# m4rch1n0/vqvae

Hardware: AMD Instinct MI355X
Metric: latents/sec through geodesic kNN+APSP+K-medoids (higher is better)
Workload: dtype f64-exact(u32 fixed point)

## Files before the change

vqvae_amd/csrc/common.hip:

```cpp
#include "geo_common.h"

#include <cstdlib>
#include <cstring>

namespace geo {

namespace {
struct OptionName { const char *name, *env; int Options::*field; };
const OptionName kOptionNames[] = {
    {"sssp_sb", "GEO_SSSP_SB", &Options::sssp_sb},
    {"sssp_act", "GEO_SSSP_ACT", &Options::sssp_act},
    {"sssp_sparse_div", "GEO_SSSP_SPARSE_DIV", &Options::sssp_sparse_div},
    {"sssp_map_div", "GEO_SSSP_MAP_DIV", &Options::sssp_map_div},
    {"sssp_group", "GEO_SSSP_GROUP", &Options::sssp_group},
    {"sssp_grouped_cap", "GEO_SSSP_GROUPED_CAP", &Options::sssp_grouped_cap},
    {"sssp_trace", "GEO_SSSP_TRACE", &Options::sssp_trace},
    {"sssp_u32", "GEO_SSSP_U32", &Options::sssp_u32},
    {"sssp_push", "GEO_SSSP_PUSH", &Options::sssp_push},
    {"sssp_order", "GEO_SSSP_ORDER", &Options::sssp_order},
    {"sssp_delta", "GEO_SSSP_DELTA", &Options::sssp_delta},
    {"sssp_push_blocks", "GEO_SSSP_PUSH_BLOCKS", &Options::sssp_push_blocks},
    {"knn_filter", "GEO_KNN_FILTER", &Options::knn_filter},
    {"kpp_grid", "GEO_KPP_GRID", &Options::kpp_grid},
    {"kpp_profile", "GEO_KPP_PROFILE", &Options::kpp_profile},
    {"jvp_mid", "GEO_JVP_MID", &Options::jvp_mid},
    {"jvp_back_valu", "GEO_JVP_BACK_VALU", &Options::jvp_back_valu},
    {"jvp_front_valu", "GEO_JVP_FRONT_VALU", &Options::jvp_front_valu},
    {"jvp_per_node", "GEO_JVP_PER_NODE", &Options::jvp_per_node},
    {"jvp_node_jacobian", "GEO_JVP_NODE_JACOBIAN", &Options::jvp_node_jacobian},
    {"jvp_pipe_grid", "GEO_JVP_PIPE_GRID", &Options::jvp_pipe_grid},
};
Options from_environment() {
    Options o;
    for (const OptionName &e : kOptionNames) {
        const char *v = getenv(e.env);
        if (!v) continue;
        if (e.field == &Options::jvp_mid) o.jvp_mid = v[0] == 'f' ? 1 : (v[0] == 'c' ? 2 : (v[0] == 'a' ? 3 : atoi(v)));
        else o.*(e.field) = atoi(v);
    }
    return o;
}
}

Options &options() {
    static Options o = from_environment();
    return o;
}

static thread_local char g_err[512] = "";

void set_error(const char *fmt, ...) {
    va_list ap;
    va_start(ap, fmt);
    vsnprintf(g_err, sizeof(g_err), fmt, ap);
    va_end(ap);
}

constexpr int SCAN_THREADS = 256;
constexpr int SCAN_ITEMS = 8;
constexpr int SCAN_TILE = SCAN_THREADS * SCAN_ITEMS;

__global__ __launch_bounds__(SCAN_THREADS) void scan_tiles_kernel(const int32_t *__restrict__ in,
                                                                 int32_t *__restrict__ out,
// ... 114 lines not shown
```

vqvae_amd/csrc/geo_common.h:

```cpp
#pragma once
#include <hip/hip_runtime.h>

#include <cstdarg>
#include <cstdint>
#include <cstdio>

#include "geo_hip.h"

namespace geo {

void set_error(const char *fmt, ...);

#define GEO_HIP_CHECK(expr)                                                                      \
    do {                                                                                         \
        hipError_t _e = (expr);                                                                  \
        if (_e != hipSuccess) {                                                                  \
            geo::set_error("%s failed: %s (%s:%d)", #expr, hipGetErrorString(_e), __FILE__, __LINE__); \
            return GEO_E_HIP;                                                                    \
        }                                                                                        \
    } while (0)

#define GEO_REQUIRE(cond, ...)              \
    do {                                    \
        if (!(cond)) {                      \
            geo::set_error(__VA_ARGS__);    \
            return GEO_E_ARG;               \
        }                                   \
    } while (0)

#define GEO_LAUNCH_CHECK() GEO_HIP_CHECK(hipGetLastError())

struct Options {
    int sssp_sb = -1, sssp_act = 1, sssp_sparse_div = -1, sssp_map_div = -1, sssp_group = 1, sssp_grouped_cap = 256,
        sssp_trace = 0, sssp_u32 = 1, sssp_push = 1 ,
        sssp_delta = 8 , sssp_order = 0 , sssp_push_blocks = 64, knn_filter = 1, kpp_grid = 256, kpp_profile = 0, jvp_mid = 0 ,
        jvp_back_valu = 0, jvp_front_valu = 0, jvp_per_node = 1 ,
        jvp_pipe_grid = 1 ,
        jvp_node_jacobian = 1 ;
};
Options &options();

static inline size_t align_up(size_t x, size_t a = 256) { return (x + a - 1) / a * a; }

struct Arena {
    char *base;
    size_t size, off;
    Arena(void *p, size_t n) : base(static_cast<char *>(p)), size(n), off(0) {}
    template <typename T>
    T *take(size_t count) {
        size_t bytes = align_up(count * sizeof(T));
        if (off + bytes > size) return nullptr;
        T *r = reinterpret_cast<T *>(base + off);
        off += bytes;
        return r;
    }
};

size_t scan_tmp_bytes(int64_t n);
int exclusive_scan_i32(const int32_t *in, int32_t *out, int64_t n, void *tmp, size_t tmp_bytes,
                       int64_t *total_host, hipStream_t stream);

static inline int grid_for(int64_t work_items, int per_block, int cap = 8192) {
    int64_t g = (work_items + per_block - 1) / per_block;
    if (g < 1) g = 1;
    if (g > cap) g = cap;
    return static_cast<int>(g);
}

}
```

vqvae_amd/csrc/jvp.hip:

```cpp
#include "geo_common.h"

#include <cmath>
#include <cstdlib>
#include <type_traits>
#include <vector>

namespace {

constexpr int TS = 32;
constexpr int NC = 128;
constexpr int MAX_BLOCKS = 4;
constexpr int FRONT_MAX_N1 = 1024;
constexpr int BACK_TS = 8;

typedef float f32x16 __attribute__((ext_vector_type(16)));
typedef __bf16 bf16x8 __attribute__((ext_vector_type(8)));
typedef unsigned short u16x8 __attribute__((ext_vector_type(8)));

struct Shape {
    int d, c0, c1, c2, co, s_out, pad3, p_out;
    int n1, n2;
    int opix_per_chunk, n_chunks;
};

// ... 855 lines not shown
#pragma unroll
    for (int lc = 0; lc < NL; ++lc) {
        const int ch = wg == 0 ? MidGeom::chunk_of(0, lc) : MidGeom::chunk_of(1, lc);
        const int op = lo == 0 ? MidGeom::opix(ch, 0) : MidGeom::opix(ch, 1);
#pragma unroll
        for (int q = 0; q < 16; ++q) {
            const int row = (q & 3) + 8 * (q >> 2) + 4 * (lane >> 5);
            const float x = accp[lc][q] + bias, t = acct[lc][q];
            if (!TONLY) pre2[(slot0 + row) * n2 + (size_t)op * c2 + co] = x;
            tpre2[(slot0 + row) * n2 + (size_t)op * c2 + co] = t;
            if (!TONLY && row < n_valid) { sx += x; sxx += (double)x * x; st_ += t; sxt += (double)x * t; }
        }
    }
    if (want_stats) {
        sx += __shfl_xor(sx, 32, 64); sxx += __shfl_xor(sxx, 32, 64);
        st_ += __shfl_xor(st_, 32, 64); sxt += __shfl_xor(sxt, 32, 64);
        if (lane < 32) { red[wave][lane][0] = sx; red[wave][lane][1] = sxx; red[wave][lane][2] = st_; red[wave][lane][3] = sxt; }
        __syncthreads();
        if (threadIdx.x < 64) {
            const int w0 = threadIdx.x >> 5, l = threadIdx.x & 31;
            double a0 = 0, a1 = 0, a2 = 0, a3 = 0;
#pragma unroll
            for (int w = 0; w < 4; ++w) { a0 += red[w0 + 2 * w][l][0]; a1 += red[w0 + 2 * w][l][1]; a2 += red[w0 + 2 * w][l][2]; a3 += red[w0 + 2 * w][l][3]; }
            double *p = partial2 + ((size_t)tile * c2 + threadIdx.x) * 4;
            p[0] = a0; p[1] = a1; p[2] = a2; p[3] = a3;
        }
    }
#ifdef GEO_MID_PROF
    { const unsigned long long t_e = __builtin_amdgcn_s_memtime();
      GEO_MP_ADD(6, t_e - mp_prev); GEO_MP_ADD(5, mp_wait); GEO_MP_ADD(7, 1); }
#endif
}

__global__ __launch_bounds__(512, 2) void mid_pipe_kernel(const float *__restrict__ pre1, const float *__restrict__ tpre1,
                                                         const NormConst *__restrict__ consts1, int consts_per_group,
                                                         int tiles_per_group, int n_tiles, int ,
                                                         const unsigned short *__restrict__ B3, const float *__restrict__ b2,
                                                         float *__restrict__ pre2, float *__restrict__ tpre2,
                                                         double *__restrict__ partial2, int want_stats, int64_t e_base,
                                                         int64_t n_edges, int batch) {
    constexpr int C1 = 128, LDK = C1 + 8, KS = C1 / 16, NL = 4, c2 = 64;
    typedef float f32x2 __attribute__((ext_vector_type(2)));
    __shared__ __attribute__((aligned(16))) unsigned short A3[2][3][2][TS][LDK];
    const int lane = threadIdx.x & 63, wave = __builtin_amdgcn_readfirstlane((int)(threadIdx.x >> 6));
    const int wq = wave & 3, wg = wave >> 2;
    constexpr int n1 = 4 * C1, n2 = 16 * c2;
    const int r = lane & 31, h = lane >> 5;
    const int k0p = 2 * lane;
    const int lo = wq >> 1, co = (wq & 1) * 32 + r;
    const float bias = b2[co];
    const unsigned v_out = (unsigned)(4 * h * n2 + co) * 4u;
    const int my_tiles = (n_tiles - (int)blockIdx.x + (int)gridDim.x - 1) / (int)gridDim.x;
    if (my_tiles <= 0) return;

    f32x16 accp[NL], acct[NL];
    auto zero_acc = [&]() {
#pragma unroll
        for (int lc = 0; lc < NL; ++lc)
#pragma unroll
            for (int i = 0; i < 16; ++i) { accp[lc][i] = 0.f; acct[lc][i] = 0.f; }
    };
    zero_acc();
    NormConst kA, kB;
    f32x2 rp[4], rt[4];
    auto load_consts = [&](int tile) {
        const NormConst *kp = consts1 + (size_t)(consts_per_group ? tile / tiles_per_group : 0) * C1 + k0p;
        kA = kp[0];
        kB = kp[1];
    };
    const unsigned v_pair = (unsigned)k0p * 4u;
    auto fetch = [&](int tile, int px, int sample0, auto ns_tag) {
        constexpr int NS = decltype(ns_tag)::value;
        const size_t tbase = (size_t)tile * TS * n1;
        const __amdgpu_buffer_rsrc_t rp_src = __builtin_amdgcn_make_buffer_rsrc(const_cast<float *>(pre1 + tbase), 0, TS * n1 * 4, 0x00020000);
        const __amdgpu_buffer_rsrc_t rt_src = __builtin_amdgcn_make_buffer_rsrc(const_cast<float *>(tpre1 + tbase), 0, TS * n1 * 4, 0x00020000);
        const int soff = (sample0 * n1 + MidGeom::pix(px) * C1) * 4;
#pragma unroll
        for (int i = 0; i < NS; ++i) {
            rp[i] = __builtin_bit_cast(f32x2, __builtin_amdgcn_raw_buffer_load_b64(rp_src, v_pair, soff + i * n1 * 4, 0));
            rt[i] = __builtin_bit_cast(f32x2, __builtin_amdgcn_raw_buffer_load_b64(rt_src, v_pair, soff + i * n1 * 4, 0));
        }
        __builtin_amdgcn_sched_group_barrier(0x020, 2 * NS, 0);
    };
    auto stage = [&](int buf, int sample0, auto ns_tag) {
        constexpr int NS = decltype(ns_tag)::value;
        unsigned w_idx = (unsigned)((buf * 3 * 2 * TS + sample0) * LDK + k0p);
        asm volatile("" : "+v"(w_idx));
        unsigned short *w = &A3[0][0][0][0][0] + w_idx;
#pragma unroll
        for (int i = 0; i < NS; ++i) {
            float a0, t0, a1, t1;
            norm_relu(kA, rp[i].x, rt[i].x, &a0, &t0);
            norm_relu(kB, rp[i].y, rt[i].y, &a1, &t1);
            unsigned wa[3], wt[3];
            split3_pair(a0, a1, wa[0], wa[1], wa[2]);
            split3_pair(t0, t1, wt[0], wt[1], wt[2]);
#pragma unroll
            for (int part = 0; part < 3; ++part) {
                *reinterpret_cast<unsigned *>(w + (part * 2 + 0) * TS * LDK + i * LDK) = wa[part];
                *reinterpret_cast<unsigned *>(w + (part * 2 + 1) * TS * LDK + i * LDK) = wt[part];
            }
        }
    };
    std::integral_constant<int, 4> HALF;
    const int s_half = 4 * wave, s_full = 8 * wq;

    bf16x8 ring[3][3];
    const unsigned b_lane = (unsigned)(h * 3 * NC * 8 + (wq * 32 + r) * 8) * 2u;
    const __amdgpu_buffer_rsrc_t b_rsrc = __builtin_amdgcn_make_buffer_rsrc(
        const_cast<unsigned short *>(B3), 0, (int)((size_t)8 * MAX_BLOCKS * C1 * NC * 3 * 2), 0x00020000);
    auto ring_init = [&]() {
        const int cb0 = wg == 0 ? MidGeom::prod_cb(0, MidGeom::pix(0), 0) : MidGeom::prod_cb(1, MidGeom::pix(0), 0);
        const int cb1 = wg == 0 ? MidGeom::prod_cb(0, MidGeom::pix(0), 1) : MidGeom::prod_cb(1, MidGeom::pix(0), 1);
#pragma unroll
        for (int part = 0; part < 3; ++part) {
            ring[0][part] = __builtin_bit_cast(bf16x8, __builtin_amdgcn_raw_buffer_load_b128(b_rsrc, b_lane, (cb0 * KS * 2 * 3 + part) * NC * 8 * 2, 0));
            ring[1][part] = __builtin_bit_cast(bf16x8, __builtin_amdgcn_raw_buffer_load_b128(b_rsrc, b_lane, (cb1 * KS * 2 * 3 + part) * NC * 8 * 2, 0));
        }
    };
    auto epilogue = [&](int tile) {
        const int group = tile / tiles_per_group;
        int64_t cnt_g = n_edges - (e_base + (int64_t)(group >> 1) * batch);
        if (cnt_g > batch) cnt_g = batch;
        const int n_valid = (int)cnt_g - (tile - group * tiles_per_group) * TS;
        const size_t tbase = (size_t)tile * TS * n2;
        const __amdgpu_buffer_rsrc_t p_dst = __builtin_amdgcn_make_buffer_rsrc(pre2 + tbase, 0, TS * n2 * 4, 0x00020000);
        const __amdgpu_buffer_rsrc_t t_dst = __builtin_amdgcn_make_buffer_rsrc(tpre2 + tbase, 0, TS * n2 * 4, 0x00020000);
        double sx = 0, sxx = 0, st_ = 0, sxt = 0;
#pragma unroll
        for (int lc = 0; lc < NL; ++lc) {
            const int ch = wg == 0 ? MidGeom::chunk_of(0, lc) : MidGeom::chunk_of(1, lc);
            const int op = lo == 0 ? MidGeom::opix(ch, 0) : MidGeom::opix(ch, 1);
#pragma unroll
            for (int q = 0; q < 16; ++q) {
                const int row = (q & 3) + 8 * (q >> 2) + 4 * h;
                const float x = accp[lc][q] + bias, t = acct[lc][q];
                const int soff = (((q & 3) + 8 * (q >> 2)) * n2 + op * c2) * 4;
                __builtin_amdgcn_raw_buffer_store_b32(__float_as_uint(x), p_dst, v_out, soff, 0);
                __builtin_amdgcn_raw_buffer_store_b32(__float_as_uint(t), t_dst, v_out, soff, 0);
                const double xd = row < n_valid ? (double)x : 0.0, td = row < n_valid ? (double)t : 0.0;
                sx += xd; sxx = fma(xd, xd, sxx); st_ += td; sxt = fma(xd, td, sxt);
            }
        }
        if (want_stats) {
            sx += __shfl_xor(sx, 32, 64); sxx += __shfl_xor(sxx, 32, 64);
            st_ += __shfl_xor(st_, 32, 64); sxt += __shfl_xor(sxt, 32, 64);
            if (lane < 32) {
                double *pp = partial2 + (((size_t)tile * 4 + (wg * 2 + (wq >> 1))) * c2 + co) * 4;
                pp[0] = sx; pp[1] = sxx; pp[2] = st_; pp[3] = sxt;
            }
        }
        zero_acc();
    };

    const unsigned short *a3 = &A3[0][0][0][0][0];
    const unsigned a_lane = (unsigned)(r * LDK + h * 8);
    constexpr unsigned A_BUF = 3u * 2u * TS * LDK;
#define GEO_PIPE_PIXEL(WGV, IPV)                                                                                       \
    mid_products<C1, false, WGV, IPV>(a3, a_lane + ((IPV) & 1) * A_BUF, b_rsrc, b_lane, accp, acct, ring)

#define GEO_PIPE_SEP() __builtin_amdgcn_sched_barrier(0)
#define GEO_STAGE_FULL(BUF, TILE, PX)                                                                                   \
    { stage(BUF, s_full, HALF); fetch(TILE, PX, s_full + 4, HALF); GEO_PIPE_SEP(); stage(BUF, s_full + 4, HALF); }

    int tile = blockIdx.x;
    load_consts(tile);
    fetch(tile, 0, s_half, HALF);
    ring_init();
    stage(0, s_half, HALF);
    if (wg == 0) fetch(tile, 1, s_full, HALF);
    else fetch(tile, 2, s_half, HALF);
    if (wg == 0) __builtin_amdgcn_s_setprio(1);
    lds_barrier();
#ifdef GEO_MID_PROF
    unsigned long long pb_prev = __builtin_amdgcn_s_memtime(), pb_wait = 0;
#define GEO_PB(slot)                                                                                                   \
    { const unsigned long long t_a = __builtin_amdgcn_s_memtime();                                                      \
      lds_barrier();                                                                                                    \
      const unsigned long long t_b = __builtin_amdgcn_s_memtime();                                                      \
      if (lane == 0 && wq == 0) { atomicAdd(&g_mid_prof[wg][1 + slot], t_a - pb_prev); atomicAdd(&g_mid_prof[wg][5], t_b - t_a);   \
                                  if (slot == 3) atomicAdd(&g_mid_prof[wg][7], 1ull); }                                 \
      pb_prev = t_b; }
#else
#define GEO_PB(slot) lds_barrier();
// ... 8 lines not shown
            GEO_PIPE_PIXEL(0, 2); GEO_PIPE_SEP(); stage(1, s_half, HALF); GEO_PB(2);
            GEO_PIPE_PIXEL(0, 3); GEO_PIPE_SEP();
            epilogue(tile);
            GEO_PIPE_SEP();
            if (has_next) { load_consts(next); fetch(next, 1, s_full, HALF); ring_init(); }
            GEO_PB(3);
            tile = next;
        }
    } else {
        for (int it = 0; it < my_tiles; ++it) {
            const int next = tile + (int)gridDim.x;
            const bool has_next = it + 1 < my_tiles;
            if (it > 0) { epilogue(tile - (int)gridDim.x); GEO_PIPE_SEP(); ring_init(); }
            GEO_PIPE_PIXEL(1, 0); GEO_PB(0);
            stage(0, s_half, HALF); fetch(tile, 3, s_half, HALF); GEO_PIPE_SEP();
            GEO_PIPE_PIXEL(1, 1); GEO_PB(1);
            stage(1, s_half, HALF);
            if (has_next) { load_consts(next); fetch(next, 0, s_full, HALF); }
            GEO_PIPE_SEP();
            GEO_PIPE_PIXEL(1, 2); GEO_PB(2);
            if (has_next) { GEO_STAGE_FULL(0, next, 0); fetch(next, 2, s_half, HALF); }
            GEO_PIPE_SEP();
            GEO_PIPE_PIXEL(1, 3); GEO_PB(3);
            tile = next;
        }
        epilogue(tile - (int)gridDim.x);
    }
#undef GEO_STAGE_FULL
#undef GEO_PIPE_SEP
#undef GEO_PB
#undef GEO_PIPE_PIXEL
}

__global__ __launch_bounds__(256) void slot_valid_kernel(int64_t e_base, int64_t n_edges, int batch, int tiles_per_group,
                                                        int64_t n_slots, int32_t *__restrict__ slot_valid) {
    for (int64_t i = (int64_t)blockIdx.x * blockDim.x + threadIdx.x; i < n_slots; i += (int64_t)gridDim.x * blockDim.x) {
        const int64_t per_group = (int64_t)tiles_per_group * TS;
        const int64_t g = i / per_group, within = i % per_group;
        const int64_t e = e_base + (g >> 1) * batch + within;
        slot_valid[i] = (within < batch && e < n_edges) ? 1 : 0;
    }
}

__global__ __launch_bounds__(256) void slot_node_kernel(const int32_t *__restrict__ src, const int32_t *__restrict__ dst,
                                                       int64_t e_base, int64_t n_edges, int batch, int tiles_per_group,
                                                       int64_t n_slots, int32_t *__restrict__ slot_node) {
    for (int64_t i = (int64_t)blockIdx.x * blockDim.x + threadIdx.x; i < n_slots; i += (int64_t)gridDim.x * blockDim.x) {
        const int64_t per_group = (int64_t)tiles_per_group * TS;
        const int64_t g = i / per_group, within = i % per_group;
        const int64_t e = e_base + (g >> 1) * batch + within;
        slot_node[i] = (within < batch && e < n_edges) ? ((g & 1) ? dst[e] : src[e]) : 0;
    }
}

__global__ __launch_bounds__(256) void back_kernel(const float *__restrict__ pre2, const float *__restrict__ tpre2,
                                                  const NormConst *__restrict__ consts2, int consts_per_group,
                                                  int slots_per_group, int c2, int co_n, int s_out, int pad3,
                                                  const float *__restrict__ W3p, const float *__restrict__ b3,
                                                  float *__restrict__ norms) {
    extern __shared__ __attribute__((aligned(16))) float smem[];
    const int n2 = 16 * c2;
    const int p_out = co_n * s_out * s_out;
    const int ldc = c2 + 4;
    const int lds_n2 = 16 * ldc;
    float *a2 = smem;
    float *ta2 = a2 + (size_t)BACK_TS * lds_n2;
// ... 63 lines not shown
}

__global__ __launch_bounds__(256) void pack_back_bf16_kernel(const float *__restrict__ w3, int c2, int co_n, int s_out,
                                                            int pad3, int np, unsigned short *__restrict__ W3b) {
    const int K = 16 * c2, P = co_n * s_out * s_out;
    const size_t total = (size_t)K * np;
    for (size_t i = (size_t)blockIdx.x * blockDim.x + threadIdx.x; i < total; i += (size_t)gridDim.x * blockDim.x) {
        const int o = (int)(i % np), k = (int)(i / np);
        float v = 0.f;
        if (o < P) {
            const int ip = k / c2, ci = k % c2, iy = ip >> 2, ix = ip & 3;
            const int co = o / (s_out * s_out), oy = (o / s_out) % s_out, ox = o % s_out;
            const int ky = oy + pad3 - 2 * iy, kx = ox + pad3 - 2 * ix;
            if (ky >= 0 && ky < 4 && kx >= 0 && kx < 4) v = w3[(((size_t)ci * co_n + co) * 4 + ky) * 4 + kx];
        }
        unsigned short q[3];
        split3(v, q[0], q[1], q[2]);
        const int kb = k >> 7, kk = k & 127, ks = kk >> 4, h = (kk >> 3) & 1, j = kk & 7;
        for (int part = 0; part < 3; ++part)
            W3b[((((size_t)kb * 3 + part) * 8 + ks) * 2 + h) * (size_t)np * 8 + (size_t)o * 8 + j] = q[part];
    }
}

template <int NT, bool GN, int MODE = 0>
__global__ __launch_bounds__(256, 2) void back_mfma_kernel(const float *__restrict__ pre2, const float *__restrict__ tpre2,
                                                       const NormConst *__restrict__ consts2, int consts_per_group,
                                                       int tiles_per_group, int co_n, int s_out,
                                                       const unsigned short *__restrict__ W3b,
                                                       const float *__restrict__ b3, float *__restrict__ norms,
                                                       const float4 *__restrict__ gs2, float *__restrict__ sg_node = nullptr,
                                                       const int32_t *__restrict__ src = nullptr,
                                                       const int32_t *__restrict__ dst = nullptr, int64_t e_base = 0,
                                                       int64_t n_edges = 0, int batch = 1, float *__restrict__ jac_node = nullptr,
                                                       int unit_d = 0) {
    constexpr int C2 = 64, KB = 128, LDK = KB + 8, NP = NT * 32;
    __shared__ __attribute__((aligned(16))) unsigned short A3[3][2][TS][LDK];
    __shared__ NormConst kc[C2];
    __shared__ float4 gsl[GN ? TS : 1][32];
    const int tile = blockIdx.x;
    const int group = tile / tiles_per_group;
    const int lane = threadIdx.x & 63, wave = threadIdx.x >> 6;
    const int n2 = 16 * C2, P = co_n * s_out * s_out;
    const size_t slot0 = (size_t)tile * TS;
    for (int c = threadIdx.x; c < C2; c += 256) kc[c] = consts2[(size_t)(consts_per_group ? group : 0) * C2 + c];
    if (GN)
        for (int i = threadIdx.x; i < TS * 32; i += 256) gsl[i >> 5][i & 31] = gs2[slot0 * 32 + i];

    f32x16 accp[NT], acct[NT];
#pragma unroll
    for (int nt = 0; nt < NT; ++nt)
#pragma unroll
        for (int i = 0; i < 16; ++i) { accp[nt][i] = 0.f; acct[nt][i] = 0.f; }

    const int r = lane & 31, h = lane >> 5;
    const int ss = threadIdx.x >> 3, k0 = (threadIdx.x & 7) * 16;
    auto edge_of = [&](int sample) -> int64_t {
        const int tg = tile - group * tiles_per_group;
        const int64_t e = e_base + (int64_t)(group >> 1) * batch + (int64_t)tg * TS + sample;
        return (tg * TS + sample >= batch || e >= n_edges) ? -1 : e;
    };
    auto node_of = [&](int sample) -> size_t {
        const int64_t e = edge_of(sample);
        return e < 0 ? 0 : (size_t)((group & 1) ? dst[e] : src[e]);
    };
    const size_t prow = MODE == 1 ? node_of(ss) : slot0 + ss;
    for (int kb = 0; kb < 8; ++kb) {
        __syncthreads();
        {
            const float *xp = pre2 + prow * n2 + (size_t)kb * KB + k0;
            const float *xt = (MODE == 2 ? pre2 : tpre2) + (slot0 + ss) * n2 + (size_t)kb * KB + k0;
#pragma unroll
            for (int k8 = 0; k8 < 16; k8 += 8) {
                u16x8 pp[3], pt[3];
#pragma unroll
                for (int k = 0; k < 8; ++k) {
                    float a, ta;
                    const int c = (k0 + k8 + k) & (C2 - 1);
                    if (GN) norm_relu_gn(gsl[GN ? ss : 0][c >> 1], kc[c].sc, kc[c].beta, xp[k8 + k], xt[k8 + k], &a, &ta);
                    else norm_relu(kc[c], xp[k8 + k], xt[k8 + k], &a, &ta);
                    unsigned short q1, q2, q3;
                    if (MODE != 1) { split3(a, q1, q2, q3); pp[0][k] = q1; pp[1][k] = q2; pp[2][k] = q3; }
                    if (MODE != 2) { split3(ta, q1, q2, q3); pt[0][k] = q1; pt[1][k] = q2; pt[2][k] = q3; }
                }
#pragma unroll
                for (int part = 0; part < 3; ++part) {
                    if (MODE != 1) *reinterpret_cast<u16x8 *>(&A3[part][0][ss][k0 + k8]) = pp[part];
                    if (MODE != 2) *reinterpret_cast<u16x8 *>(&A3[part][1][ss][k0 + k8]) = pt[part];
                }
            }
        }
        __syncthreads();
#pragma unroll
        for (int kq = 0; kq < 2; ++kq) {
            const int ks = wave * 2 + kq;
            bf16x8 ap[3], at[3];
#pragma unroll
            for (int part = 0; part < 3; ++part) {
                if (MODE != 1) ap[part] = *reinterpret_cast<const bf16x8 *>(&A3[part][0][r][ks * 16 + h * 8]);
                if (MODE != 2) at[part] = *reinterpret_cast<const bf16x8 *>(&A3[part][1][r][ks * 16 + h * 8]);
            }
#pragma unroll
            for (int nt = 0; nt < NT; ++nt) {
                bf16x8 b[3];
#pragma unroll
                for (int part = 0; part < 3; ++part)
                    b[part] = *reinterpret_cast<const bf16x8 *>(
                        W3b + ((((size_t)kb * 3 + part) * 8 + ks) * 2 + h) * (size_t)NP * 8 + (size_t)(nt * 32 + r) * 8);
                if (MODE != 1) accp[nt] = __builtin_amdgcn_mfma_f32_32x32x16_bf16(ap[2], b[0], accp[nt], 0, 0, 0);
                if (MODE != 2) acct[nt] = __builtin_amdgcn_mfma_f32_32x32x16_bf16(at[2], b[0], acct[nt], 0, 0, 0);
                if (MODE != 1) accp[nt] = __builtin_amdgcn_mfma_f32_32x32x16_bf16(ap[0], b[2], accp[nt], 0, 0, 0);
                if (MODE != 2) acct[nt] = __builtin_amdgcn_mfma_f32_32x32x16_bf16(at[0], b[2], acct[nt], 0, 0, 0);
                if (MODE != 1) accp[nt] = __builtin_amdgcn_mfma_f32_32x32x16_bf16(ap[1], b[1], accp[nt], 0, 0, 0);
                if (MODE != 2) acct[nt] = __builtin_amdgcn_mfma_f32_32x32x16_bf16(at[1], b[1], acct[nt], 0, 0, 0);
                if (MODE != 1) accp[nt] = __builtin_amdgcn_mfma_f32_32x32x16_bf16(ap[1], b[0], accp[nt], 0, 0, 0);
                if (MODE != 2) acct[nt] = __builtin_amdgcn_mfma_f32_32x32x16_bf16(at[1], b[0], acct[nt], 0, 0, 0);
                if (MODE != 1) accp[nt] = __builtin_amdgcn_mfma_f32_32x32x16_bf16(ap[0], b[1], accp[nt], 0, 0, 0);
                if (MODE != 2) acct[nt] = __builtin_amdgcn_mfma_f32_32x32x16_bf16(at[0], b[1], acct[nt], 0, 0, 0);
                if (MODE != 1) accp[nt] = __builtin_amdgcn_mfma_f32_32x32x16_bf16(ap[0], b[0], accp[nt], 0, 0, 0);
                if (MODE != 2) acct[nt] = __builtin_amdgcn_mfma_f32_32x32x16_bf16(at[0], b[0], acct[nt], 0, 0, 0);
            }
        }
    }
    float *red = reinterpret_cast<float *>(&A3[0][0][0][0]);
    const int row = threadIdx.x >> 3, c4 = (threadIdx.x & 7) * 4;
    const size_t nrow = MODE == 1 ? node_of(row) : slot0 + row;
    float *jrow = nullptr;
    if (MODE == 1 && jac_node) {
        const int64_t e = edge_of(row);
        if (e >= 0) jrow = jac_node + (nrow * unit_d + (size_t)(e % unit_d)) * NP;
    }
    double sumsq = 0.0;
#pragma unroll
    for (int nt = 0; nt < NT; ++nt) {
        __syncthreads();
#pragma unroll
        for (int q = 0; q < 16; ++q) {
            const int rr = (q & 3) + 8 * (q >> 2) + 4 * (lane >> 5);
            if (MODE != 1) red[((wave * 2 + 0) * 32 + rr) * 33 + (lane & 31)] = accp[nt][q];
            if (MODE != 2) red[((wave * 2 + 1) * 32 + rr) * 33 + (lane & 31)] = acct[nt][q];
        }
        __syncthreads();
#pragma unroll
        for (int c = 0; c < 4; ++c) {
            const int o = nt * 32 + c4 + c;
            if (o < P) {
                float x = b3[o / (s_out * s_out)], t = 0.f;
#pragma unroll
                for (int w = 0; w < 4; ++w) {
                    if (MODE != 1) x += red[((w * 2 + 0) * 32 + row) * 33 + c4 + c];
                    if (MODE != 2) t += red[((w * 2 + 1) * 32 + row) * 33 + c4 + c];
                }
                const float sg = MODE == 1 ? sg_node[nrow * NP + o] : 1.0f / (1.0f + expf(-x));
                if (MODE == 2) sg_node[nrow * NP + o] = sg;
                const float j = t * sg * (1.0f - sg);
                if (MODE == 1 && jrow) jrow[o] = j;
                sumsq += (double)(j * j);
            }
        }
    }
    sumsq += __shfl_xor(sumsq, 1, 64);
    sumsq += __shfl_xor(sumsq, 2, 64);
    sumsq += __shfl_xor(sumsq, 4, 64);
    if (MODE != 2 && (threadIdx.x & 7) == 0) norms[slot0 + row] = (float)sqrt(sumsq);
}

__global__ __launch_bounds__(256) void combine_kernel(const float *__restrict__ norms, int64_t e_base, int64_t e_count,
                                                     int batch, int slots_per_group, float *__restrict__ len_out) {
    for (int64_t i = (int64_t)blockIdx.x * blockDim.x + threadIdx.x; i < e_count; i += (int64_t)gridDim.x * blockDim.x) {
        const int64_t chunk = i / batch, within = i % batch;
        const float a = norms[(chunk * 2 + 0) * slots_per_group + within];
        const float b = norms[(chunk * 2 + 1) * slots_per_group + within];
        len_out[e_base + i] = 0.5f * (a + b);
    }
}

__global__ __launch_bounds__(256) void pair_edges_kernel(int64_t n_nodes, int d, int64_t n_pseudo, int32_t *__restrict__ src,
                                                        int32_t *__restrict__ dst) {
    for (int64_t i = (int64_t)blockIdx.x * blockDim.x + threadIdx.x; i < n_pseudo; i += (int64_t)gridDim.x * blockDim.x) {
        const int64_t a = 2 * (i / d), b = a + 1 < n_nodes ? a + 1 : n_nodes - 1;
        src[i] = (int32_t)a;
        dst[i] = (int32_t)b;
    }
}

__global__ __launch_bounds__(256) void jacobian_lengths_kernel(const float *__restrict__ z, const int32_t *__restrict__ src,
                                                              const int32_t *__restrict__ dst, int64_t n_edges, int d, int p_out,
                                                              int np, const float *__restrict__ jac_node,
                                                              float *__restrict__ len_out) {
    const int64_t gid = (int64_t)blockIdx.x * 256 + threadIdx.x;
    const int l = (int)(gid & 15);
    int64_t e = gid >> 4;
    const bool live = e < n_edges;
    if (!live) e = n_edges - 1;
    const int64_t a = src[e], b = dst[e];
    float dz[16];
#pragma unroll
// ... 272 lines not shown
        const bool front_mfma = s.d > 16 && s.n1 % 32 == 0 && geo::options().jvp_front_valu == 0;
        if (s.d <= 16) { if (geo::options().jvp_front_valu == 2 && s.n1 % 32 == 0 && !unit_d) GEO_FRONT_MFMA(16); else GEO_FRONT(16); }
        else if (s.d <= 32) { if (front_mfma) GEO_FRONT_MFMA(32); else GEO_FRONT(32); }
        else { if (front_mfma) GEO_FRONT_MFMA(64); else GEO_FRONT(64); }
#undef GEO_FRONT_MFMA
#undef GEO_FRONT
        GEO_LAUNCH_CHECK();
        if (batch_stats) {
            finalize_batch_kernel<<<geo::grid_for(p_groups * s.c1, 256), 256, 0, stream>>>(
                part1, pl.tiles_per_group, 1, 4, s.c1, e_base, n_edges, batch, dc->g1, dc->be1, dc->eps, k1, (int)p_groups,
                track ? stats : nullptr);
            if (track)
                running_update_kernel<<<(unsigned)((s.c1 + 7) / 8), 256, 0, stream>>>(stats, (int)p_groups, s.c1, dc->momentum,
                                                                          const_cast<float *>(dc->rm1), const_cast<float *>(dc->rv1));
            GEO_LAUNCH_CHECK();
        }
        if (gs1) {
            group_stats_kernel<<<geo::grid_for(p_slots * 32, 256), 256, 0, stream>>>(pre1, tpre1, p_slots, 4, s.c1, 32,
                                                                                    dc->eps, gs1);
            GEO_LAUNCH_CHECK();
        }
        const dim3 mgrid((unsigned)p_tiles, (unsigned)s.n_chunks);
#define GEO_MID(C1V)                                                                                               \
    mid_kernel<C1V><<<mgrid, 256, 0, stream>>>(pre1, tpre1, k1, batch_stats ? 1 : 0, pl.tiles_per_group, tab,       \
                                               s.opix_per_chunk, s.c2, B2p, dc->b2, pre2, tpre2, part2,             \
                                               batch_stats ? 1 : 0, slot_valid)
#define GEO_MID3(C1V)                                                                                              \
    mid_bf16_kernel<C1V><<<mgrid, 256, 0, stream>>>(pre1, tpre1, k1, batch_stats ? 1 : 0, pl.tiles_per_group, tab,  \
                                                    s.opix_per_chunk, s.c2, B3, dc->b2, pre2, tpre2, part2,        \
                                                    batch_stats ? 1 : 0, slot_valid)
        const bool mid_all = mid_split && s.n_chunks == 8 && s.opix_per_chunk == 2 && s.c1 >= 32 &&
                             mid_opt != 2;
        const bool mid_pipe = mid_all && !per_node && !gs1 && s.c1 == 128 && s.c2 == 64 && mid_opt != 3;
        if (mid_all && per_node) {
#define GEO_MIDA_T(C1V, GNV)                                                                                       \
    mid_all_kernel<C1V, GNV, true><<<(unsigned)p_tiles, 512, 0, stream>>>(pre1, tpre1, k1, 0, pl.tiles_per_group,       \
                                                                          s.c2, B3, dc->b2, pre2, tpre2, part2, 0,     \
                                                                          slot_valid, gs1, e_base, n_edges, batch)
            if (gs1) { if (s.c1 == 128) GEO_MIDA_T(128, true); else if (s.c1 == 64) GEO_MIDA_T(64, true); else GEO_MIDA_T(32, true); }
            else if (s.c1 == 128) GEO_MIDA_T(128, false);
            else if (s.c1 == 64) GEO_MIDA_T(64, false);
            else GEO_MIDA_T(32, false);
#undef GEO_MIDA_T
        } else if (mid_pipe) {
            static int n_cu = 0;
            if (n_cu == 0) {
                int devid = 0;
                hipDeviceProp_t prop;
                GEO_HIP_CHECK(hipGetDevice(&devid));
                GEO_HIP_CHECK(hipGetDeviceProperties(&prop, devid));
                n_cu = prop.multiProcessorCount > 0 ? prop.multiProcessorCount : 256;
            }
            const int per_cu = geo::options().jvp_pipe_grid > 0 ? geo::options().jvp_pipe_grid : 1;
            const unsigned pgrid = (unsigned)std::min<int64_t>(p_tiles, (int64_t)n_cu * per_cu);
            mid_pipe_kernel<<<pgrid, 512, 0, stream>>>(pre1, tpre1, k1, batch_stats ? 1 : 0, pl.tiles_per_group, (int)p_tiles,
                                                       s.c2, B3, dc->b2, pre2, tpre2, part2, batch_stats ? 1 : 0, e_base,
                                                       n_edges, batch);
        } else if (mid_all) {
#define GEO_MIDA(C1V, GNV)                                                                                         \
    mid_all_kernel<C1V, GNV><<<(unsigned)p_tiles, 512, 0, stream>>>(pre1, tpre1, k1, batch_stats ? 1 : 0,           \
                                                                    pl.tiles_per_group, s.c2, B3, dc->b2,           \
                                                                    pre2, tpre2, part2, batch_stats ? 1 : 0,        \
                                                                    slot_valid, gs1, e_base, n_edges, batch)
            if (gs1) {
                if (s.c1 == 128) GEO_MIDA(128, true);
                else if (s.c1 == 64) GEO_MIDA(64, true);
                else GEO_MIDA(32, true);
            } else if (s.c1 == 128) GEO_MIDA(128, false);
            else if (s.c1 == 64) GEO_MIDA(64, false);
            else GEO_MIDA(32, false);
#undef GEO_MIDA
        } else if (mid_split) {
            if (s.c1 == 128) GEO_MID3(128);
            else if (s.c1 == 64) GEO_MID3(64);
            else GEO_MID3(32);
        } else {
            if (s.c1 == 128) GEO_MID(128);
            else if (s.c1 == 64) GEO_MID(64);
            else GEO_MID(32);
        }
#undef GEO_MID3
#undef GEO_MID
        GEO_LAUNCH_CHECK();
        if (batch_stats) {
            finalize_batch_kernel<<<geo::grid_for(p_groups * s.c2, 256), 256, 0, stream>>>(
                part2, pl.tiles_per_group, mid_pipe ? 4 : (mid_all ? 1 : 16), 16, s.c2, e_base, n_edges, batch, dc->g2, dc->be2, dc->eps, k2, (int)p_groups,
                track ? stats : nullptr);
            if (track)
                running_update_kernel<<<(unsigned)((s.c2 + 7) / 8), 256, 0, stream>>>(stats, (int)p_groups, s.c2, dc->momentum,
                                                                          const_cast<float *>(dc->rm2), const_cast<float *>(dc->rv2));
            GEO_LAUNCH_CHECK();
        }
        if (gs2 && per_node) {
            slot_node_kernel<<<geo::grid_for(p_slots, 256), 256, 0, stream>>>(src, dst, e_base, n_edges, batch, pl.tiles_per_group,
                                                                             p_slots, slot_valid);
            group_stats_kernel<<<geo::grid_for(p_slots * 32, 256), 256, 0, stream>>>(pre2_node, tpre2, p_slots, 16, s.c2, 32,
                                                                                    dc->eps, gs2, slot_valid);
            GEO_LAUNCH_CHECK();
        } else if (gs2) {
            group_stats_kernel<<<geo::grid_for(p_slots * 32, 256), 256, 0, stream>>>(pre2, tpre2, p_slots, 16, s.c2, 32,
                                                                                    dc->eps, gs2);
            GEO_LAUNCH_CHECK();
        }
#define GEO_BACK(NTV, GNV)                                                                                         \
    back_mfma_kernel<NTV, GNV><<<(unsigned)p_tiles, 256, 0, stream>>>(pre2, tpre2, k2, batch_stats ? 1 : 0,         \
                                                                      pl.tiles_per_group, s.co, s.s_out, W3b,       \
                                                                      dc->b3, norms, gs2)
#define GEO_BACK_T(NTV, GNV)                                                                                       \
    back_mfma_kernel<NTV, GNV, 1><<<(unsigned)p_tiles, 256, 0, stream>>>(pre2_node, tpre2, k2, 0, pl.tiles_per_group, s.co, \
                                                                         s.s_out, W3b, dc->b3, norms, gs2, sg_node, src,   \
                                                                         dst, e_base, n_edges, batch, jac_node, unit_d)
        if (per_node && back_nt == 1) { if (gs2) GEO_BACK_T(1, true); else GEO_BACK_T(1, false); }
        else if (per_node) { if (gs2) GEO_BACK_T(6, true); else GEO_BACK_T(6, false); }
#undef GEO_BACK_T
        else if (back_mfma && back_nt == 1) { if (gs2) GEO_BACK(1, true); else GEO_BACK(1, false); }
        else if (back_mfma) { if (gs2) GEO_BACK(6, true); else GEO_BACK(6, false); }
#undef GEO_BACK
        else
            back_kernel<<<(unsigned)(p_slots / BACK_TS), 256, back_lds, stream>>>(
                pre2, tpre2, k2, batch_stats ? 1 : 0, pl.slots_per_group, s.c2, s.co, s.s_out, s.pad3, W3p, dc->b3, norms);
        GEO_LAUNCH_CHECK();
        if (len_out) {
            combine_kernel<<<geo::grid_for(e_count, 256), 256, 0, stream>>>(norms, e_base, e_count, batch,
                                                                            pl.slots_per_group, len_out);
            GEO_LAUNCH_CHECK();
        }
    }
    return GEO_OK;
}

struct JacobianPlan {
    int64_t n_pseudo;
    size_t np, extra_bytes, bytes;
};

bool node_jacobian_plan(const geo_decoder_desc *dc, int64_t n_nodes, int64_t n_edges, int batch, JacobianPlan *jp) {
    const geo::Options &o = geo::options();
    Shape s;
    if (!dc || n_nodes <= 0 || n_edges <= 0 || !make_shape(dc, &s)) return false;
    if (o.jvp_node_jacobian == 0 || o.jvp_per_node == 0 || o.jvp_back_valu || o.jvp_mid == 1 || o.jvp_mid == 2) return false;
    if (dc->norm == 1 && dc->bn_train) return false;
    if (s.d > 16 || s.c1 % 16 != 0 || s.c1 < 32 || s.c2 != 64 || s.n_chunks != 8 || s.opix_per_chunk != 2) return false;
    const int back_nt = (s.p_out + 31) / 32;
    if (back_nt != 1 && back_nt != 6) return false;
    if (o.jvp_node_jacobian == 1 && 4 * n_edges < 3 * n_nodes * s.d) return false;
// ... 78 lines not shown
```

Measured before the change: 2.102 million.

## Deduplicate repeated start-node rows in JVP mid and back stages

Adds a run-detection kernel that finds consecutive edges sharing the same source node, then computes the primal mid/back activations once per unique start node instead of once per edge. The generic pipe kernel handles only end-node tiles, and a new mid_start kernel processes the compacted start rows plus a per-tile tangent pass that gathers primal values through a row map. The back stage is split into three launches (end side, compact start primal, start tangent via row_map). This removes redundant work when edges are sorted by source, at the cost of extra launches, scratch space reused from part1/pre1, and a single-block-per-chunk serial loop for compact rows.

```diff
diff --git a/vqvae_amd/csrc/common.hip b/vqvae_amd/csrc/common.hip
--- a/vqvae_amd/csrc/common.hip
+++ b/vqvae_amd/csrc/common.hip
@@ -29,6 +29,7 @@
     {"jvp_per_node", "GEO_JVP_PER_NODE", &Options::jvp_per_node},
     {"jvp_node_jacobian", "GEO_JVP_NODE_JACOBIAN", &Options::jvp_node_jacobian},
     {"jvp_pipe_grid", "GEO_JVP_PIPE_GRID", &Options::jvp_pipe_grid},
+    {"jvp_start_dedup", "GEO_JVP_START_DEDUP", &Options::jvp_start_dedup},
 };
 Options from_environment() {
     Options o;
diff --git a/vqvae_amd/csrc/geo_common.h b/vqvae_amd/csrc/geo_common.h
--- a/vqvae_amd/csrc/geo_common.h
+++ b/vqvae_amd/csrc/geo_common.h
@@ -36,7 +36,8 @@
         sssp_delta = 8 , sssp_order = 0 , sssp_push_blocks = 64, knn_filter = 1, kpp_grid = 256, kpp_profile = 0, jvp_mid = 0 ,
         jvp_back_valu = 0, jvp_front_valu = 0, jvp_per_node = 1 ,
         jvp_pipe_grid = 1 ,
-        jvp_node_jacobian = 1 ;
+        jvp_node_jacobian = 1 ,
+        jvp_start_dedup = 1 ;
 };
 Options &options();
 
diff --git a/vqvae_amd/csrc/jvp.hip b/vqvae_amd/csrc/jvp.hip
--- a/vqvae_amd/csrc/jvp.hip
+++ b/vqvae_amd/csrc/jvp.hip
@@ -911,6 +911,21 @@
 #endif
 }
 
+struct Bn2Sums { double sx = 0, sxx = 0, st = 0, sxt = 0; };
+__device__ __forceinline__ void bn2_add(Bn2Sums &a, float x, float t, bool live) {
+    const double xd = live ? (double)x : 0.0, td = live ? (double)t : 0.0;
+    a.sx += xd; a.sxx = fma(xd, xd, a.sxx); a.st += td; a.sxt = fma(xd, td, a.sxt);
+}
+__device__ __forceinline__ void bn2_store(Bn2Sums a, double *__restrict__ partial2, int tile, int wslot, int co, int lane) {
+    a.sx += __shfl_xor(a.sx, 32, 64); a.sxx += __shfl_xor(a.sxx, 32, 64);
+    a.st += __shfl_xor(a.st, 32, 64); a.sxt += __shfl_xor(a.sxt, 32, 64);
+    if (lane < 32) {
+        double *pp = partial2 + (((size_t)tile * 4 + wslot) * 64 + co) * 4;
+        pp[0] = a.sx; pp[1] = a.sxx; pp[2] = a.st; pp[3] = a.sxt;
+    }
+}
+
+template <bool END_ONLY>
 __global__ __launch_bounds__(512, 2) void mid_pipe_kernel(const float *__restrict__ pre1, const float *__restrict__ tpre1,
                                                          const NormConst *__restrict__ consts1, int consts_per_group,
                                                          int tiles_per_group, int n_tiles, int ,
@@ -942,7 +957,9 @@
     zero_acc();
     NormConst kA, kB;
     f32x2 rp[4], rt[4];
+    auto phys = [&](int t) { return END_ONLY ? ((t / tiles_per_group) * 2 + 1) * tiles_per_group + t % tiles_per_group : t; };
     auto load_consts = [&](int tile) {
+        tile = phys(tile);
         const NormConst *kp = consts1 + (size_t)(consts_per_group ? tile / tiles_per_group : 0) * C1 + k0p;
         kA = kp[0];
         kB = kp[1];
@@ -950,7 +967,7 @@
     const unsigned v_pair = (unsigned)k0p * 4u;
     auto fetch = [&](int tile, int px, int sample0, auto ns_tag) {
         constexpr int NS = decltype(ns_tag)::value;
-        const size_t tbase = (size_t)tile * TS * n1;
+        const size_t tbase = (size_t)phys(tile) * TS * n1;
         const __amdgpu_buffer_rsrc_t rp_src = __builtin_amdgcn_make_buffer_rsrc(const_cast<float *>(pre1 + tbase), 0, TS * n1 * 4, 0x00020000);
         const __amdgpu_buffer_rsrc_t rt_src = __builtin_amdgcn_make_buffer_rsrc(const_cast<float *>(tpre1 + tbase), 0, TS * n1 * 4, 0x00020000);
         const int soff = (sample0 * n1 + MidGeom::pix(px) * C1) * 4;
@@ -998,6 +1015,7 @@
         }
     };
     auto epilogue = [&](int tile) {
+        tile = phys(tile);
         const int group = tile / tiles_per_group;
         int64_t cnt_g = n_edges - (e_base + (int64_t)(group >> 1) * batch);
         if (cnt_g > batch) cnt_g = batch;
@@ -1005,7 +1023,7 @@
         const size_t tbase = (size_t)tile * TS * n2;
         const __amdgpu_buffer_rsrc_t p_dst = __builtin_amdgcn_make_buffer_rsrc(pre2 + tbase, 0, TS * n2 * 4, 0x00020000);
         const __amdgpu_buffer_rsrc_t t_dst = __builtin_amdgcn_make_buffer_rsrc(tpre2 + tbase, 0, TS * n2 * 4, 0x00020000);
-        double sx = 0, sxx = 0, st_ = 0, sxt = 0;
+        Bn2Sums sums;
 #pragma unroll
         for (int lc = 0; lc < NL; ++lc) {
             const int ch = wg == 0 ? MidGeom::chunk_of(0, lc) : MidGeom::chunk_of(1, lc);
@@ -1017,18 +1035,10 @@
                 const int soff = (((q & 3) + 8 * (q >> 2)) * n2 + op * c2) * 4;
                 __builtin_amdgcn_raw_buffer_store_b32(__float_as_uint(x), p_dst, v_out, soff, 0);
                 __builtin_amdgcn_raw_buffer_store_b32(__float_as_uint(t), t_dst, v_out, soff, 0);
-                const double xd = row < n_valid ? (double)x : 0.0, td = row < n_valid ? (double)t : 0.0;
-                sx += xd; sxx = fma(xd, xd, sxx); st_ += td; sxt = fma(xd, td, sxt);
-            }
-        }
-        if (want_stats) {
-            sx += __shfl_xor(sx, 32, 64); sxx += __shfl_xor(sxx, 32, 64);
-            st_ += __shfl_xor(st_, 32, 64); sxt += __shfl_xor(sxt, 32, 64);
-            if (lane < 32) {
-                double *pp = partial2 + (((size_t)tile * 4 + (wg * 2 + (wq >> 1))) * c2 + co) * 4;
-                pp[0] = sx; pp[1] = sxx; pp[2] = st_; pp[3] = sxt;
-            }
-        }
+                bn2_add(sums, x, t, row < n_valid);
+            }
+        }
+        if (want_stats) bn2_store(sums, partial2, tile, wg * 2 + (wq >> 1), co, lane);
         zero_acc();
     };
 
@@ -1103,6 +1113,194 @@
 #undef GEO_PIPE_PIXEL
 }
 
+__global__ __launch_bounds__(256) void start_runs_kernel(const int32_t *__restrict__ src, int64_t e_base, int64_t n_edges, int batch,
+                                                        int slots_per_group, int32_t *__restrict__ row_map, int32_t *__restrict__ rep,
+                                                        int32_t *__restrict__ n_compact) {
+    __shared__ int wsum[4];
+    __shared__ int carry_s;
+    const int chunk = blockIdx.x;
+    const size_t g0 = (size_t)chunk * 2 * slots_per_group;
+    const int lane = threadIdx.x & 63, wave = threadIdx.x >> 6;
+    int carry = 0;
+    for (int w0 = 0; w0 < slots_per_group; w0 += 256) {
+        const int within = w0 + (int)threadIdx.x;
+        const int64_t e = e_base + (int64_t)chunk * batch + within;
+        const bool valid = within < slots_per_group && within < batch && e < n_edges;
+        const bool head = valid && (within == 0 || src[e] != src[e - 1]);
+        const unsigned long long m = __ballot(head);
+        const int below = __popcll(m & ((1ull << lane) - 1ull));
+        if (lane == 0) wsum[wave] = __popcll(m);
+        __syncthreads();
+        int before = carry, total = carry;
+        for (int w = 0; w < 4; ++w) { if (w < wave) before += wsum[w]; total += wsum[w]; }
+        const int k = before + below + (head ? 1 : 0) - 1;
+        if (within < slots_per_group) {
+            row_map[g0 + within] = (int32_t)(g0 + (valid ? k : 0));
+            if (head) rep[g0 + k] = (int32_t)(g0 + within);
+        }
+        carry = total;
+        __syncthreads();
+    }
+    if (threadIdx.x == 0) { carry_s = carry; n_compact[chunk] = carry; }
+    __syncthreads();
+    const int cnt = carry_s, padded = (cnt + TS - 1) / TS * TS;
+    for (int k = cnt + (int)threadIdx.x; k < padded; k += 256) rep[g0 + k] = (int32_t)g0;
+}
+
+template <bool TT>
+__global__ __launch_bounds__(512, 2) void mid_start_kernel(const float *__restrict__ pre1, const float *__restrict__ tpre1,
+                                                          const NormConst *__restrict__ consts1, int tiles_per_group,
+                                                          const unsigned short *__restrict__ B3, const float *__restrict__ b2,
+                                                          float *__restrict__ pre2, float *__restrict__ tpre2,
+                                                          double *__restrict__ partial2, const int32_t *__restrict__ row_map,
+                                                          const int32_t *__restrict__ rep, const int32_t *__restrict__ n_compact,
+                                                          int64_t e_base, int64_t n_edges, int batch) {
+    constexpr int C1 = 128, LDK = C1 + 8, KS = C1 / 16, NL = 4, c2 = 64, n1 = 4 * C1, n2 = 16 * c2;
+    typedef float f32x2 __attribute__((ext_vector_type(2)));
+    __shared__ __attribute__((aligned(16))) unsigned short A3[2][3][2][TS][LDK];
+    const int chunk = blockIdx.y, group = 2 * chunk;
+    const int ncomp = TT ? 0 : n_compact[chunk];
+    auto run = [&](int item) {
+    const int lt0 = 2 * item;
+    const bool live1 = TT ? lt0 + 1 < tiles_per_group : (lt0 + 1) * TS < ncomp;
+    const int tile0 = group * tiles_per_group + lt0, tile1 = live1 ? tile0 + 1 : tile0;
+    const int lane = threadIdx.x & 63, wave = __builtin_amdgcn_readfirstlane((int)(threadIdx.x >> 6));
+    const int wq = wave & 3, wg = wave >> 2;
+    const int r = lane & 31, h = lane >> 5;
+    f32x16 accp[NL], acct[NL];
+#pragma unroll
+    for (int lc = 0; lc < NL; ++lc)
+#pragma unroll
+        for (int i = 0; i < 16; ++i) { accp[lc][i] = 0.f; acct[lc][i] = 0.f; }
+
+    const int k0p = 2 * lane, s0p = 4 * wave;
+    const NormConst *kp = consts1 + (size_t)group * C1 + k0p;
+    const NormConst kA = kp[0], kB = kp[1];
+    size_t xrow[2][4];
+#pragma unroll
+    for (int i = 0; i < 4; ++i) {
+        const size_t s0 = (size_t)tile0 * TS + s0p + i, s1 = (size_t)tile1 * TS + s0p + i;
+        xrow[0][i] = TT ? s0 : (size_t)__builtin_amdgcn_readfirstlane(rep[s0]);
+        xrow[1][i] = TT ? s1 : (size_t)__builtin_amdgcn_readfirstlane(rep[s1]);
+    }
+    f32x2 rx[2][4], rt[2][4];
+    auto fetch = [&](int nx) {
+#pragma unroll
+        for (int hh = 0; hh < 2; ++hh)
+#pragma unroll
+            for (int i = 0; i < 4; ++i) {
+                const size_t off = xrow[hh][i] * n1 + (size_t)MidGeom::pix(nx) * C1 + k0p;
+                rx[hh][i] = *reinterpret_cast<const f32x2 *>(pre1 + off);
+                if (TT) rt[hh][i] = *reinterpret_cast<const f32x2 *>(tpre1 + off);
+            }
+    };
+    fetch(0);
+    auto stage_px = [&](int buf, int nx) {
+#pragma unroll
+        for (int hh = 0; hh < 2; ++hh)
+#pragma unroll
+            for (int i = 0; i < 4; ++i) {
+                float a0, t0, a1, t1;
+                norm_relu(kA, rx[hh][i].x, TT ? rt[hh][i].x : 0.f, &a0, &t0);
+                norm_relu(kB, rx[hh][i].y, TT ? rt[hh][i].y : 0.f, &a1, &t1);
+                unsigned w[3];
+                if (TT) split3_pair(t0, t1, w[0], w[1], w[2]);
+                else split3_pair(a0, a1, w[0], w[1], w[2]);
+#pragma unroll
+                for (int part = 0; part < 3; ++part) *reinterpret_cast<unsigned *>(&A3[buf][part][hh][s0p + i][k0p]) = w[part];
+            }
+        if (nx < 4) {
+            fetch(nx);
+            __builtin_amdgcn_sched_group_barrier(0x020, TT ? 16 : 8, 0);
+        }
+    };
+    bf16x8 ring[3][3];
+    const unsigned b_lane = (unsigned)(h * 3 * NC * 8 + (wq * 32 + r) * 8) * 2u;
+    const __amdgpu_buffer_rsrc_t b_rsrc = __builtin_amdgcn_make_buffer_rsrc(
+        const_cast<unsigned short *>(B3), 0, (int)((size_t)8 * MAX_BLOCKS * C1 * NC * 3 * 2), 0x00020000);
+    {
+        const int cb0 = wg == 0 ? MidGeom::prod_cb(0, MidGeom::pix(0), 0) : MidGeom::prod_cb(1, MidGeom::pix(0), 0);
+        const int cb1 = wg == 0 ? MidGeom::prod_cb(0, MidGeom::pix(0), 1) : MidGeom::prod_cb(1, MidGeom::pix(0), 1);
+#pragma unroll
+        for (int part = 0; part < 3; ++part) {
+            ring[0][part] = __builtin_bit_cast(bf16x8, __builtin_amdgcn_raw_buffer_load_b128(b_rsrc, b_lane, (cb0 * KS * 2 * 3 + part) * NC * 8 * 2, 0));
+            ring[1][part] = __builtin_bit_cast(bf16x8, __builtin_amdgcn_raw_buffer_load_b128(b_rsrc, b_lane, (cb1 * KS * 2 * 3 + part) * NC * 8 * 2, 0));
+        }
+    }
+    stage_px(0, 1);
+    if (wg == 1) __builtin_amdgcn_s_setprio(1);
+    lds_barrier();
+    const unsigned short *a3 = &A3[0][0][0][0][0];
+    const unsigned a_lane = (unsigned)(r * LDK + h * 8);
+    constexpr unsigned A_BUF = 3u * 2u * TS * LDK;
+#define GEO_MID_PIXEL(WGV, IPV) mid_products<C1, false, WGV, IPV>(a3, a_lane + ((IPV) & 1) * A_BUF, b_rsrc, b_lane, accp, acct, ring)
+    if (wg == 0) {
+        GEO_MID_PIXEL(0, 0); stage_px(1, 2); lds_barrier();
+        GEO_MID_PIXEL(0, 1); stage_px(0, 3); lds_barrier();
+        GEO_MID_PIXEL(0, 2); stage_px(1, 4); lds_barrier();
+        GEO_MID_PIXEL(0, 3);
+    } else {
+        stage_px(1, 2); GEO_MID_PIXEL(1, 0); lds_barrier();
+        stage_px(0, 3); GEO_MID_PIXEL(1, 1); lds_barrier();
+        stage_px(1, 4); GEO_MID_PIXEL(1, 2); lds_barrier();
+        GEO_MID_PIXEL(1, 3);
+    }
+#undef GEO_MID_PIXEL
+
+    const int lo = wq >> 1, co = (wq & 1) * 32 + r;
+    const float bias = TT ? 0.f : b2[co];
+    float *dst = TT ? tpre2 : pre2;
+#pragma unroll
+    for (int hh = 0; hh < 2; ++hh) {
+        if (hh == 1 && !live1) break;
+        const size_t tbase = (size_t)(hh ? tile1 : tile0) * TS;
+#pragma unroll
+        for (int lc = 0; lc < NL; ++lc) {
+            const int ch = wg == 0 ? MidGeom::chunk_of(0, lc) : MidGeom::chunk_of(1, lc);
+            const int op = lo == 0 ? MidGeom::opix(ch, 0) : MidGeom::opix(ch, 1);
+#pragma unroll
+            for (int q = 0; q < 16; ++q) {
+                const int row = (q & 3) + 8 * (q >> 2) + 4 * h;
+                const float v = hh ? acct[lc][q] : accp[lc][q];
+                dst[(tbase + row) * n2 + (size_t)op * c2 + co] = TT ? v : v + bias;
+            }
+        }
+    }
+    if (TT) {
+        int64_t cnt_g = n_edges - (e_base + (int64_t)chunk * batch);
+        if (cnt_g > batch) cnt_g = batch;
+#pragma unroll
+        for (int hh = 0; hh < 2; ++hh) {
+            if (hh == 1 && !live1) break;
+            const int tile = hh ? tile1 : tile0;
+            const size_t tbase = (size_t)tile * TS;
+            const int n_valid = (int)cnt_g - (tile - group * tiles_per_group) * TS;
+            Bn2Sums sums;
+#pragma unroll
+            for (int lc = 0; lc < NL; ++lc) {
+                const int ch = wg == 0 ? MidGeom::chunk_of(0, lc) : MidGeom::chunk_of(1, lc);
+                const int op = lo == 0 ? MidGeom::opix(ch, 0) : MidGeom::opix(ch, 1);
+#pragma unroll
+                for (int q = 0; q < 16; ++q) {
+                    const int row = (q & 3) + 8 * (q >> 2) + 4 * h;
+                    const float x = pre2[(size_t)row_map[tbase + row] * n2 + (size_t)op * c2 + co];
+                    bn2_add(sums, x, hh ? acct[lc][q] : accp[lc][q], row < n_valid);
+                }
+            }
+            bn2_store(sums, partial2, tile, wg * 2 + (wq >> 1), co, lane);
+        }
+    }
+    };
+    if (TT) {
+        run((int)blockIdx.x);
+    } else {
+        for (int item = 0; 2 * item * TS < ncomp; ++item) {
+            if (item > 0) { __builtin_amdgcn_s_setprio(0); __syncthreads(); }
+            run(item);
+        }
+    }
+}
+
 __global__ __launch_bounds__(256) void slot_valid_kernel(int64_t e_base, int64_t n_edges, int batch, int tiles_per_group,
                                                         int64_t n_slots, int32_t *__restrict__ slot_valid) {
     for (int64_t i = (int64_t)blockIdx.x * blockDim.x + threadIdx.x; i < n_slots; i += (int64_t)gridDim.x * blockDim.x) {
@@ -1232,12 +1430,19 @@
                                                        const int32_t *__restrict__ src = nullptr,
                                                        const int32_t *__restrict__ dst = nullptr, int64_t e_base = 0,
                                                        int64_t n_edges = 0, int batch = 1, float *__restrict__ jac_node = nullptr,
-                                                       int unit_d = 0) {
+                                                       int unit_d = 0, const int32_t *__restrict__ row_map = nullptr,
+                                                       const int32_t *__restrict__ n_compact = nullptr, int side_only = 0) {
     constexpr int C2 = 64, KB = 128, LDK = KB + 8, NP = NT * 32;
     __shared__ __attribute__((aligned(16))) unsigned short A3[3][2][TS][LDK];
     __shared__ NormConst kc[C2];
     __shared__ float4 gsl[GN ? TS : 1][32];
-    const int tile = blockIdx.x;
+    const int n_iter = MODE == 2 && n_compact ? (n_compact[blockIdx.x] + TS - 1) / TS : 1;
+    for (int it = 0; it < n_iter; ++it) {
+    if (it > 0) __syncthreads();
+    const int tile = MODE == 2 && n_compact ? (int)blockIdx.x * 2 * tiles_per_group + it
+                   : side_only ? (((int)blockIdx.x / tiles_per_group) * 2 + side_only - 1) * tiles_per_group +
+                                     (int)blockIdx.x % tiles_per_group
+                               : (int)blockIdx.x;
     const int group = tile / tiles_per_group;
     const int lane = threadIdx.x & 63, wave = threadIdx.x >> 6;
     const int n2 = 16 * C2, P = co_n * s_out * s_out;
@@ -1263,7 +1468,7 @@
         const int64_t e = edge_of(sample);
         return e < 0 ? 0 : (size_t)((group & 1) ? dst[e] : src[e]);
     };
-    const size_t prow = MODE == 1 ? node_of(ss) : slot0 + ss;
+    const size_t prow = MODE == 1 ? (row_map ? (size_t)row_map[slot0 + ss] : node_of(ss)) : slot0 + ss;
     for (int kb = 0; kb < 8; ++kb) {
         __syncthreads();
         {
@@ -1323,7 +1528,7 @@
     }
     float *red = reinterpret_cast<float *>(&A3[0][0][0][0]);
     const int row = threadIdx.x >> 3, c4 = (threadIdx.x & 7) * 4;
-    const size_t nrow = MODE == 1 ? node_of(row) : slot0 + row;
+    const size_t nrow = MODE == 1 ? (row_map ? (size_t)row_map[slot0 + row] : node_of(row)) : slot0 + row;
     float *jrow = nullptr;
     if (MODE == 1 && jac_node) {
         const int64_t e = edge_of(row);
@@ -1362,6 +1567,7 @@
     sumsq += __shfl_xor(sumsq, 2, 64);
     sumsq += __shfl_xor(sumsq, 4, 64);
     if (MODE != 2 && (threadIdx.x & 7) == 0) norms[slot0 + row] = (float)sqrt(sumsq);
+    }
 }
 
 __global__ __launch_bounds__(256) void combine_kernel(const float *__restrict__ norms, int64_t e_base, int64_t e_count,
@@ -1700,6 +1906,18 @@
         const bool mid_all = mid_split && s.n_chunks == 8 && s.opix_per_chunk == 2 && s.c1 >= 32 &&
                              mid_opt != 2;
         const bool mid_pipe = mid_all && !per_node && !gs1 && s.c1 == 128 && s.c2 == 64 && mid_opt != 3;
+        const size_t np_back = (size_t)back_nt * 32;
+        const bool dedup = batch_stats && src && dst && mid_pipe && back_mfma && !jac_node && !gs2 &&
+                           geo::options().jvp_start_dedup != 0 && (2 * slots + groups) * 4 <= tiles * s.n1 * 4 * 8 &&
+                           np_back <= (size_t)s.n1;
+        int32_t *row_map = reinterpret_cast<int32_t *>(part1), *rep = row_map + slots, *n_compact = rep + slots;
+        float *sg_compact = pre1;
+        const int64_t side_tiles = nch * pl.tiles_per_group;
+        if (dedup) {
+            start_runs_kernel<<<(unsigned)nch, 256, 0, stream>>>(src, e_base, n_edges, batch, pl.slots_per_group, row_map, rep,
+                                                                 n_compact);
+            GEO_LAUNCH_CHECK();
+        }
         if (mid_all && per_node) {
 #define GEO_MIDA_T(C1V, GNV)                                                                                       \
     mid_all_kernel<C1V, GNV, true><<<(unsigned)p_tiles, 512, 0, stream>>>(pre1, tpre1, k1, 0, pl.tiles_per_group,       \
@@ -1720,10 +1938,23 @@
                 n_cu = prop.multiProcessorCount > 0 ? prop.multiProcessorCount : 256;
             }
             const int per_cu = geo::options().jvp_pipe_grid > 0 ? geo::options().jvp_pipe_grid : 1;
-            const unsigned pgrid = (unsigned)std::min<int64_t>(p_tiles, (int64_t)n_cu * per_cu);
-            mid_pipe_kernel<<<pgrid, 512, 0, stream>>>(pre1, tpre1, k1, batch_stats ? 1 : 0, pl.tiles_per_group, (int)p_tiles,
-                                                       s.c2, B3, dc->b2, pre2, tpre2, part2, batch_stats ? 1 : 0, e_base,
-                                                       n_edges, batch);
+            const int64_t pipe_tiles = dedup ? side_tiles : p_tiles;
+            const unsigned pgrid = (unsigned)std::min<int64_t>(pipe_tiles, (int64_t)n_cu * per_cu);
+#define GEO_PIPE(EO)                                                                                               \
+    mid_pipe_kernel<EO><<<pgrid, 512, 0, stream>>>(pre1, tpre1, k1, batch_stats ? 1 : 0, pl.tiles_per_group, (int)pipe_tiles, \
+                                                   s.c2, B3, dc->b2, pre2, tpre2, part2, batch_stats ? 1 : 0, e_base,  \
+                                                   n_edges, batch)
+            if (dedup) GEO_PIPE(true);
+            else GEO_PIPE(false);
+#undef GEO_PIPE
+            if (dedup) {
+                const dim3 sgrid((unsigned)((pl.tiles_per_group + 1) / 2), (unsigned)nch);
+                mid_start_kernel<false><<<dim3(1, (unsigned)nch), 512, 0, stream>>>(pre1, tpre1, k1, pl.tiles_per_group, B3, dc->b2, pre2, tpre2,
+                                                                   part2, row_map, rep, n_compact, e_base, n_edges, batch);
+                GEO_LAUNCH_CHECK();
+                mid_start_kernel<true><<<sgrid, 512, 0, stream>>>(pre1, tpre1, k1, pl.tiles_per_group, B3, dc->b2, pre2, tpre2,
+                                                                  part2, row_map, rep, n_compact, e_base, n_edges, batch);
+            }
         } else if (mid_all) {
 #define GEO_MIDA(C1V, GNV)                                                                                         \
     mid_all_kernel<C1V, GNV><<<(unsigned)p_tiles, 512, 0, stream>>>(pre1, tpre1, k1, batch_stats ? 1 : 0,           \
@@ -1778,7 +2009,21 @@
     back_mfma_kernel<NTV, GNV, 1><<<(unsigned)p_tiles, 256, 0, stream>>>(pre2_node, tpre2, k2, 0, pl.tiles_per_group, s.co, \
                                                                          s.s_out, W3b, dc->b3, norms, gs2, sg_node, src,   \
                                                                          dst, e_base, n_edges, batch, jac_node, unit_d)
-        if (per_node && back_nt == 1) { if (gs2) GEO_BACK_T(1, true); else GEO_BACK_T(1, false); }
+#define GEO_BACK_D(NTV)                                                                                            \
+    do {                                                                                                            \
+    back_mfma_kernel<NTV, false, 0><<<(unsigned)side_tiles, 256, 0, stream>>>(                                      \
+        pre2, tpre2, k2, 1, pl.tiles_per_group, s.co, s.s_out, W3b, dc->b3, norms, nullptr, nullptr, nullptr, nullptr, \
+        0, 0, 1, nullptr, 0, nullptr, nullptr, 2);                                                                  \
+    back_mfma_kernel<NTV, false, 2><<<(unsigned)nch, 256, 0, stream>>>(                                      \
+        pre2, tpre2, k2, 1, pl.tiles_per_group, s.co, s.s_out, W3b, dc->b3, norms, nullptr, sg_compact, nullptr,     \
+        nullptr, 0, 0, 1, nullptr, 0, nullptr, n_compact, 1);                                                       \
+    back_mfma_kernel<NTV, false, 1><<<(unsigned)side_tiles, 256, 0, stream>>>(                                      \
+        pre2, tpre2, k2, 1, pl.tiles_per_group, s.co, s.s_out, W3b, dc->b3, norms, nullptr, sg_compact, nullptr,     \
+        nullptr, 0, 0, 1, nullptr, 0, row_map, nullptr, 1);                                                        \
+    } while (0)
+        if (dedup) { if (back_nt == 1) GEO_BACK_D(1); else GEO_BACK_D(6); }
+#undef GEO_BACK_D
+        else if (per_node && back_nt == 1) { if (gs2) GEO_BACK_T(1, true); else GEO_BACK_T(1, false); }
         else if (per_node) { if (gs2) GEO_BACK_T(6, true); else GEO_BACK_T(6, false); }
 #undef GEO_BACK_T
         else if (back_mfma && back_nt == 1) { if (gs2) GEO_BACK(1, true); else GEO_BACK(1, false); }
```

Measured after the change: 2.300 million (median of 6 runs). 9.4% higher.
